# Yeicor/sdf-viewer

Measured on AMD Instinct MI355X. Metric: Mvoxels/s grid fill + Mrays/s sphere-trace @1080p, demo SDF, higher is better.
Workload: dtype f32

## Files before the change

### include/sdfgrid.h

```cpp
#ifndef SDFGRID_H
#define SDFGRID_H

#include <stddef.h>
#include <stdint.h>

#ifdef __cplusplus
extern "C" {
#endif

#define SDFV_ABI_VERSION 5

typedef enum sdfv_status {
    SDFV_OK = 0,
    SDFV_ERR_INVALID_ARGUMENT = -1,
    SDFV_ERR_UNKNOWN_SDF = -2,
    SDFV_ERR_HIP = -3,
    SDFV_ERR_NO_DEVICE = -4,
    SDFV_ERR_COMM = -5
} sdfv_status;

typedef struct sdfv_sample {
    float distance;
    float color[3];
    float metallic;
// ... 111 lines not shown
int  sdfv_camera_look_at(sdfv_camera *cam, const float eye[3], const float target[3], const float up[3],
                         float fovy_degrees, float aspect, float z_near, float z_far);


int sdfv_grid_init(const sdfv_grid *grid, float *tex0, float *tex1, void *stream);

int sdfv_grid_init_unvisited(const sdfv_grid *grid, uint32_t step, float *tex0, float *tex1, float *dist, void *stream);
int sdfv_grid_init_unvisited_ex(const sdfv_grid *grid, uint32_t step, float *tex0, float *tex1, float *dist, uint32_t flags,
                                void *stream);

int sdfv_fill_grid(const sdfv_demo_params *params, uint32_t sdf_id, const sdfv_grid *grid,
                   float *tex0, float *tex1, void *stream);

int sdfv_fill_grid_commit(const sdfv_demo_params *params, uint32_t sdf_id, const sdfv_grid *grid, float *tex0,
                          float *tex1, float *dist, void *stream);

#define SDFV_PASS_FRESH_GRID 1u
#define SDFV_PASS_SAME_LOAD  2u
#define SDFV_PASS_VIRGIN_GRID 4u
#define SDFV_PASS_VOLUME_INTERLEAVED 8u
#define SDFV_PASS_EXPECT_NOOP 16u
int sdfv_fill_grid_pass_ex(const sdfv_demo_params *params, uint32_t sdf_id, const sdfv_grid *grid, uint32_t step,
                           const float *changed_box, float *tex0, float *tex1, float *dist, uint32_t flags, void *stream);

int sdfv_pack_samples(const sdfv_grid *grid, uint64_t index_base, const uint32_t *indices, const sdfv_sample *samples, size_t n,
                      float *tex0, float *tex1, float *dist, uint32_t flags, void *stream);

size_t sdfv_emit_update_points_scratch_bytes(uint64_t n);
int sdfv_emit_update_points(const sdfv_grid *grid, uint32_t step, uint64_t cursor, uint64_t n, const float *changed_box,
                            const float *dist, uint32_t flags, float *points, uint32_t *indices, uint32_t *count, void *scratch,
// ... 284 lines not shown
```

### sdf-viewer_amd/__init__.py

```python
import ctypes as C
import os

import sys
import warnings

_hip_already_up = "torch" in sys.modules and getattr(sys.modules["torch"], "cuda", None) is not None \
    and sys.modules["torch"].cuda.is_initialized()
if "GPU_MAX_HW_QUEUES" not in os.environ:
    if _hip_already_up:
        warnings.warn("sdf-viewer_amd imported after the HIP runtime initialised: GPU_MAX_HW_QUEUES keeps its default "
                      "(4); the multi-GPU fill step may serialise its streams (DESIGN.md 6)", RuntimeWarning)
    else:
        os.environ["GPU_MAX_HW_QUEUES"] = "8"

import torch

from . import _capi
from ._capi import (Camera, DemoParams, Grid, Light, MarchAux, RenderParams, Sample, SdfvError, check, f3, lib,
                    MATERIAL_BRICK, MATERIAL_NORMAL, SDF_CUBE, SDF_DEMO, SDF_SPHERE)

AIR_DIST = lib.sdfv_air_dist()
AUX_FLOATS = C.sizeof(MarchAux) // 4


# ... 54 lines not shown
def _dev_ptr(t, what):
    if not (isinstance(t, torch.Tensor) and t.is_cuda and t.is_contiguous() and t.dtype == torch.float32):
        raise TypeError(f"{what} must be a contiguous float32 CUDA(HIP) tensor")
    return C.c_void_p(t.data_ptr())


def grid_init(grid, tex0, tex1, stream=None):
    check(lib.sdfv_grid_init(C.byref(grid), _dev_ptr(tex0, "tex0"), _dev_ptr(tex1, "tex1"), _stream_ptr(stream)))


def grid_init_unvisited(grid, step, tex0, tex1, dist=None, stream=None, flags=0):
    check(lib.sdfv_grid_init_unvisited_ex(C.byref(grid), int(step), _dev_ptr(tex0, "tex0"), _dev_ptr(tex1, "tex1"),
                                          None if dist is None else _dev_ptr(dist, "dist"), int(flags), _stream_ptr(stream)))


def fill_grid(params, grid, tex0, tex1, sdf_id=SDF_DEMO, stream=None, dist=None):
    assert tex0.numel() == slab_voxels(grid) * 4 and tex1.numel() == slab_voxels(grid) * 4
    assert dist is None or dist.numel() == slab_voxels(grid)
    check(lib.sdfv_fill_grid_commit(C.byref(params), sdf_id, C.byref(grid), _dev_ptr(tex0, "tex0"),
                                    _dev_ptr(tex1, "tex1"), None if dist is None else _dev_ptr(dist, "dist"),
                                    _stream_ptr(stream)))


def fill_grid_pass(params, grid, step, tex0, tex1, changed_box=None, sdf_id=SDF_DEMO, stream=None, dist=None, flags=0):
    box = None if changed_box is None else (C.c_float * 6)(*[float(x) for x in changed_box])
    check(lib.sdfv_fill_grid_pass_ex(C.byref(params), sdf_id, C.byref(grid), int(step), box, _dev_ptr(tex0, "tex0"),
                                     _dev_ptr(tex1, "tex1"), None if dist is None else _dev_ptr(dist, "dist"), int(flags),
                                     _stream_ptr(stream)))


def pack_samples(grid, samples, tex0, tex1, indices=None, index_base=0, dist=None, flags=0, stream=None):
    assert samples.is_cuda and samples.dtype == torch.float32 and samples.is_contiguous() and samples.shape[-1] == 7
    n = samples.numel() // 7
# ... 255 lines not shown
```

### sdf-viewer_amd/_capi.py

```python
import ctypes as C
import os

_HERE = os.path.dirname(os.path.abspath(__file__))
LIB_PATH = os.environ.get("SDFGRID_LIBRARY") or os.path.join(_HERE, "libsdfgrid.so")


class SdfvError(RuntimeError):
    def __init__(self, code, message):
        super().__init__(f"libsdfgrid error {code}: {message}")
        self.code = code


class Sample(C.Structure):
    _fields_ = [("distance", C.c_float), ("color", C.c_float * 3), ("metallic", C.c_float),
                ("roughness", C.c_float), ("occlusion", C.c_float)]


class DemoParams(C.Structure):
    _fields_ = [("cube_half_side", C.c_float), ("cube_material", C.c_uint32),
                ("sphere_radius", C.c_float), ("sphere_material", C.c_uint32),
                ("max_distance_custom_material", C.c_float), ("disable_sphere", C.c_uint32)]


class Grid(C.Structure):
# ... 75 lines not shown
    "sdfv_render_params_default": (None, [C.POINTER(RenderParams), C.POINTER(Grid)]),
    "sdfv_camera_look_at": (C.c_int, [C.POINTER(Camera), C.POINTER(C.c_float), C.POINTER(C.c_float),
                                      C.POINTER(C.c_float), C.c_float, C.c_float, C.c_float, C.c_float]),
    "sdfv_grid_init": (C.c_int, [C.POINTER(Grid), C.c_void_p, C.c_void_p, C.c_void_p]),
    "sdfv_grid_init_unvisited": (C.c_int, [C.POINTER(Grid), C.c_uint32, C.c_void_p, C.c_void_p, C.c_void_p, C.c_void_p]),
    "sdfv_grid_init_unvisited_ex": (C.c_int, [C.POINTER(Grid), C.c_uint32, C.c_void_p, C.c_void_p, C.c_void_p, C.c_uint32, C.c_void_p]),
    "sdfv_fill_grid": (C.c_int, [C.POINTER(DemoParams), C.c_uint32, C.POINTER(Grid), C.c_void_p, C.c_void_p,
                                 C.c_void_p]),
    "sdfv_pack_samples": (C.c_int, [C.POINTER(Grid), C.c_uint64, C.c_void_p, C.c_void_p, C.c_size_t, C.c_void_p, C.c_void_p,
                                    C.c_void_p, C.c_uint32, C.c_void_p]),
    "sdfv_emit_update_points_scratch_bytes": (C.c_size_t, [C.c_uint64]),
    "sdfv_emit_update_points": (C.c_int, [C.POINTER(Grid), C.c_uint32, C.c_uint64, C.c_uint64, C.POINTER(C.c_float), C.c_void_p,
                                          C.c_uint32, C.c_void_p, C.c_void_p, C.c_void_p, C.c_void_p, C.c_size_t, C.c_void_p]),
    "sdfv_fill_grid_commit": (C.c_int, [C.POINTER(DemoParams), C.c_uint32, C.POINTER(Grid), C.c_void_p, C.c_void_p,
                                        C.c_void_p, C.c_void_p]),
    "sdfv_fill_grid_pass_ex": (C.c_int, [C.POINTER(DemoParams), C.c_uint32, C.POINTER(Grid), C.c_uint32,
                                         C.POINTER(C.c_float), C.c_void_p, C.c_void_p, C.c_void_p, C.c_uint32, C.c_void_p]),
    "sdfv_sample_points": (C.c_int, [C.POINTER(DemoParams), C.c_uint32, C.c_void_p, C.c_size_t, C.c_int,
                                     C.c_void_p, C.c_void_p]),
    "sdfv_normal_points": (C.c_int, [C.POINTER(DemoParams), C.c_uint32, C.c_void_p, C.c_size_t, C.c_float,
                                     C.c_int, C.c_void_p, C.c_void_p]),
    "sdfv_commit_distance": (C.c_int, [C.POINTER(Grid), C.c_void_p, C.c_void_p, C.c_void_p]),
    "sdfv_commit_pairs": (C.c_int, [C.POINTER(Grid), C.c_void_p, C.c_void_p, C.c_void_p]),
    "sdfv_band_rows": (C.c_uint32, [C.c_uint32, C.c_uint32, C.c_uint32]),
    "sdfv_band_rows_ex": (C.c_uint32, [C.c_uint32, C.c_uint32, C.c_uint32, C.c_uint32]),
    "sdfv_march_volume_advice": (C.c_int, [C.POINTER(Grid), C.POINTER(C.c_uint32)]),
    "sdfv_commit_interleaved": (C.c_int, [C.POINTER(Grid), C.c_void_p, C.c_void_p, C.c_void_p]),
    "sdfv_fill_grid_host": (C.c_int, [C.POINTER(DemoParams), C.c_uint32, C.POINTER(Grid), C.c_void_p, C.c_void_p]),
    "sdfv_sample_points_host": (C.c_int, [C.POINTER(DemoParams), C.c_uint32, C.c_void_p, C.c_size_t, C.c_int,
                                          C.c_void_p]),
# ... 132 lines not shown
```

### sdf-viewer_amd/csrc/api_fill.hip

```cpp
#include <cstring>

#include "api_internal.h"
#include "fill_kernels.h"
#include "ingest_kernels.h"
#include "program_kernels.h"

using namespace sdfv;

namespace {

template <typename Args>
void set_grid_fill_args(Args& a, const sdfv_grid& g, float* tex0, float* tex1, float* dist = nullptr, uint32_t dist_ilv = 0) {
    a.W = g.dims[0];
    a.H = g.dims[1];
    a.z_begin = g.z_begin;
    a.slab_d = g.z_end - g.z_begin;
    sdfv::set_voxel_coords(a, g);
    a.air_dist = air_dist();
    a.tex0 = reinterpret_cast<float4*>(tex0);
    a.tex1 = reinterpret_cast<float4*>(tex1);
    a.dist = dist;
    a.dist_ilv = dist_ilv;
    a.srgb_round = g_options.ext_srgb_quant;
}
// ... 135 lines not shown
                                              grid->z_end - grid->z_begin, step, air_dist(),
                                              (flags & SDFV_PASS_VOLUME_INTERLEAVED) ? 1u : 0u, (hipStream_t)stream));
}

int sdfv_fill_grid_commit(const sdfv_demo_params* params, uint32_t sdf_id, const sdfv_grid* grid, float* tex0,
                          float* tex1, float* dist, void* stream) {
    if (int rc = check_params(params, sdf_id)) return rc;
    if (int rc = check_grid(grid)) return rc;
    if (int rc = check_textures(tex0, tex1)) return rc;
    if (int rc = check_word_aligned("dist", dist)) return rc;
    if (int rc = need_device()) return rc;
    sdfv::FillArgs a = make_fill_args(*params, sdf_id, *grid, tex0, tex1);
    a.dist = dist;
    if (int rc = check_one_launch(a)) return rc;
    SDFV_HIP_RETURN(sdfv::launch_fill_dense(a, fill_launch_config(dist != nullptr), (hipStream_t)stream));
}

int sdfv_fill_grid(const sdfv_demo_params* params, uint32_t sdf_id, const sdfv_grid* grid, float* tex0, float* tex1,
                   void* stream) {
    return sdfv_fill_grid_commit(params, sdf_id, grid, tex0, tex1, nullptr, stream);
}

int sdfv_fill_grid_pass_ex(const sdfv_demo_params* params, uint32_t sdf_id, const sdfv_grid* grid, uint32_t step,
                           const float* changed_box, float* tex0, float* tex1, float* dist, uint32_t flags, void* stream) {
    if (int rc = check_params(params, sdf_id)) return rc;
    if (int rc = check_grid(grid)) return rc;
    if (int rc = need_textures(tex0, tex1)) return rc;
    if (step == 0 || (step & (step - 1))) return set_error(SDFV_ERR_INVALID_ARGUMENT, "step %u is not a power of two", step);
    if (flags & ~(SDFV_PASS_FRESH_GRID | SDFV_PASS_SAME_LOAD | SDFV_PASS_VIRGIN_GRID | SDFV_PASS_VOLUME_INTERLEAVED | SDFV_PASS_EXPECT_NOOP))
        return set_error(SDFV_ERR_INVALID_ARGUMENT, "unknown pass flags 0x%x", flags);
// ... 119 lines not shown
```

### sdf-viewer_amd/csrc/demo_sdf_device.h

```cpp
#pragma once

#include <hip/hip_runtime.h>
#include <stdint.h>

#include "../../include/sdfgrid.h"

namespace sdfv {

__device__ __forceinline__ float fmod_pow2(float a, float m, float inv_m) {
    return a - truncf(a * inv_m) * m;
}

struct Mat {
    float r, g, b, metallic, roughness, occlusion;
};

__device__ __forceinline__ Mat brick_tex2d(float u, float v) {
    const float BRICK_WIDTH = 0.5f, BRICK_HEIGHT = 0.25f;
    const float max_cement_displacement = 0.2f / 2.0f * 0.25f;
    float row_num = v * 4.0f;
    float brick_offset = floorf(row_num) * 0.25f;
    float bx = fmod_pow2(fabsf(u + brick_offset), BRICK_WIDTH, 2.0f);
    float by = fmod_pow2(fabsf(v), BRICK_HEIGHT, 4.0f);
    bool cement = bx < max_cement_displacement || bx > BRICK_WIDTH - max_cement_displacement ||
// ... 249 lines not shown
        distance = fmaxf(d_box, -d_sph);
        float inter = fabsf(d_box) - fabsf(d_sph);
        if (fabsf(inter) <= prm.max_distance_custom_material) {
            m = PackedSet<Cfg::kRound>::kCustom;
        } else if (inter < 0.0f) {
            m = cube_packed<Cfg>(prm, px, py, pz, d_box, lut);
        } else {
            m = sphere_packed<Cfg>(prm, px, py, pz, len, d_sph, lut);
        }
    }
    t0.x = clamp01_rust(1e-1f + distance);
    t0.y = m.lr; t0.z = m.lg; t0.w = m.lb;
    t1.x = m.metallic; t1.y = m.roughness; t1.z = m.occlusion; t1.w = air_dist;
}

__device__ __forceinline__ float voxel_coord(uint32_t idx, float dim_minus_1, float bb_size, float bb_min) {
    float p = (float)idx;
    p = p / dim_minus_1;
    p = p * bb_size;
    p = p + bb_min;
    return p;
}


__device__ __forceinline__ void cube_normal(const sdfv_demo_params& prm, float px, float py, float pz,
                                            float& nx, float& ny, float& nz) {
    float side = prm.cube_half_side;
    nx = fabsf(px) > side ? signum_f32(px) : 0.0f;
    ny = fabsf(py) > side ? signum_f32(py) : 0.0f;
    nz = fabsf(pz) > side ? signum_f32(pz) : 0.0f;
// ... 45 lines not shown
```

### sdf-viewer_amd/csrc/fill_kernels.h

```cpp
#pragma once

#include <hip/hip_runtime.h>
#include <stdint.h>

#include "../../include/sdfgrid.h"

namespace sdfv {

struct FillArgs {
    sdfv_demo_params prm;
    uint32_t sdf_id;
    uint32_t W, H, D;
    uint32_t z_begin;
    uint32_t slab_d;
    float dm1[3];
    float bb_size[3];
    float bb_min[3];
    float air_dist;
    uint32_t x_chunks;
    unsigned long long w_magic;
    uint32_t z_step;
    float4* tex0;
    float4* tex1;
    float* dist;
// ... 39 lines not shown
    uint32_t no_adaptive;
    uint32_t stream_loads;
    uint64_t index_limit;
    uint32_t n_visited;
    DivU32 div_nx, div_ny, div_w;
};

struct FillLaunch {
    bool nontemporal;
    bool force_flat = false, force_rows = false;
    bool force_paired = false, force_pairrows = false;
    bool xcd_pairing = false;
};

hipError_t launch_fill_dense(const FillArgs& a, const FillLaunch& cfg, hipStream_t stream);
struct OrderedBlocks {
    uint32_t per_slice, total;
};
OrderedBlocks ordered_blocks(const FillArgs& a);
hipError_t launch_fill_dense_ordered(const FillArgs& a, uint32_t block_begin, uint32_t block_end, hipStream_t stream);
struct CopySegments {
    const float4* src[4];
    float4* dst[4];
    uint32_t n[4];
    float* r_out[4];
};
hipError_t launch_copy_segments(const CopySegments& c, hipStream_t stream);
hipError_t launch_fill_slices(const FillArgs& a, hipStream_t stream);
hipError_t launch_fill_pass(const FillArgs& a, const PassArgs& p, const FillLaunch& dense_cfg, hipStream_t stream);
hipError_t launch_commit_distance(const float* tex0, float* dist, uint64_t n_voxels, hipStream_t stream);
// ... 8 lines not shown
```

### sdf-viewer_amd/csrc/fill_kernels.hip

```cpp
#include "fill_kernels.h"

#include "kernel_common.h"

namespace sdfv {

namespace {

template <typename T>
__device__ __forceinline__ T load_scan(const T* p, uint32_t stream) {
    return stream ? load_once(p) : *p;
}

template <int TX, bool NT, typename Cfg, bool ORDERED = false>
__global__ __launch_bounds__(kBlock) void fill_dense_kernel(FillArgs a) {
    if (!ORDERED) signal_launch_started(a);
    dense_fill_rows<TX, NT, ORDERED>(a, DemoFillEval<Cfg>{a.prm, a.sdf_id});
}

template <bool NT, typename Cfg>
__global__ __launch_bounds__(kBlock) void fill_dense_pairrows_kernel(FillArgs a) {
    __shared__ float s_lut[256];
    __shared__ float2 s_yz[2];
    const uint32_t tid = threadIdx.x;
    signal_launch_started(a);
    const uint32_t pair = a.x_chunks == 1 ? blockIdx.x : blockIdx.x / a.x_chunks;
    const uint32_t chunk = blockIdx.x - pair * a.x_chunks;
    const LdsLut lut = stage_srgb_lut(s_lut);
    if (tid < 2) s_yz[tid] = stage_row_yz(a, 2 * pair + tid);
    __syncthreads();
    const uint32_t x = chunk * kBlock + tid;
    const float px = voxel_coord(x, a.dm1[0], a.bb_size[0], a.bb_min[0]);
// ... 376 lines not shown
}

template <int TX, bool NT>
hipError_t launch_dense_cfg(const FillArgs& args, hipStream_t stream) {
    constexpr int TY = kBlock / TX;
    FillArgs a = args;
    a.x_chunks = (a.W + TX - 1) / TX;
    const uint64_t n_rows = (uint64_t)a.H * a.slab_d;
    const uint64_t blocks = a.x_chunks * ((n_rows + TY - 1) / TY);
    if (blocks > 0x7fffffffull) return hipErrorInvalidValue;
    dim3 grid((uint32_t)blocks, 1, 1);
    SDFV_LAUNCH_CFG(a, (fill_dense_kernel<TX, NT, Cfg>), grid, dim3(kBlock), 0, stream, a);
    return hipGetLastError();
}

template <bool NT>
hipError_t launch_dense_pairrows(const FillArgs& args, hipStream_t stream) {
    FillArgs a = args;
    a.x_chunks = a.W / kBlock;
    const uint64_t blocks = a.x_chunks * ((uint64_t)a.H * a.slab_d / 2);
    if (blocks > 0x7fffffffull) return hipErrorInvalidValue;
    SDFV_LAUNCH_CFG(a, (fill_dense_pairrows_kernel<NT, Cfg>), dim3((uint32_t)blocks), dim3(kBlock), 0, stream, a);
    return hipGetLastError();
}

template <bool NT>
hipError_t launch_dense_ilv_paired(const FillArgs& args, hipStream_t stream) {
    FillArgs a = args;
    a.x_chunks = a.W / kBlock;
    const uint64_t units = a.x_chunks * ((uint64_t)a.H * a.slab_d / 2);
// ... 110 lines not shown
            return cfg.nontemporal ? launch_dense_ilv_paired<true>(a, stream) : launch_dense_ilv_paired<false>(a, stream);
        if (a.W % kBlock == 0 && (cfg.force_pairrows || (a.W >= 2 * kBlock && !cfg.force_rows)))
            return cfg.nontemporal ? launch_dense_pairrows<true>(a, stream) : launch_dense_pairrows<false>(a, stream);
        return a.W <= 64 ? launch_dense_tx<64>(a, cfg, stream) : launch_dense_tx<128>(a, cfg, stream);
    }
    const uint32_t chunk = a.W <= 64 ? 64 : (a.W <= 128 ? 128 : 256);
    const bool lanes_full = a.W % chunk == 0;
    const uint64_t n_vox = (uint64_t)a.W * a.H * a.slab_d;
    if (n_vox < (1ull << 32) && (cfg.force_flat || (!lanes_full && !cfg.force_rows)))
        return cfg.nontemporal ? launch_dense_flat<true>(a, stream) : launch_dense_flat<false>(a, stream);
    if (a.W <= 64) return launch_dense_tx<64>(a, cfg, stream);
    if (a.W <= 128) return launch_dense_tx<128>(a, cfg, stream);
    return launch_dense_tx<256>(a, cfg, stream);
}

static DivU32 make_div(uint32_t d) {
    DivU32 v;
    v.pow2 = d != 0 && (d & (d - 1)) == 0;
    v.shift = 0;
    while (v.pow2 && (1u << v.shift) < d) ++v.shift;
    v.magic = d > 1 ? (~0ull / d) + 1ull : 0ull;
    return v;
}

hipError_t launch_fill_pass(const FillArgs& a, const PassArgs& pass, const FillLaunch& dense_cfg, hipStream_t stream) {
    PassArgs p = pass;
    if (p.virgin) p.fresh = p.all_required = 1;
    for (int i = 0; i < 3; ++i) {
        p.approx_scale[i] = a.dm1[i] > 0.0f ? a.bb_size[i] / a.dm1[i] : 0.0f;
        p.approx_margin[i] = 64.0f * 1.1920929e-7f * (fabsf(a.bb_size[i]) + fabsf(a.bb_min[i]));
// ... 121 lines not shown
```

### sdf-viewer_amd/csrc/kernel_common.h

```cpp
#pragma once

#include <hip/hip_runtime.h>
#include <stdint.h>

#include "demo_sdf_device.h"
#include "fill_kernels.h"

namespace sdfv {

constexpr int kBlock = 256;

typedef float v4f __attribute__((ext_vector_type(4)));

namespace {
__constant__ float c_srgb_lut[256] = {
#include "srgb_lut.inc"
};
}

struct LdsLut {
    const float* p;
    __device__ __forceinline__ float operator[](uint32_t i) const { return p[i]; }
};

// ... 160 lines not shown
            store_texel<NT>(a.tex1 + o, v1);
            if (a.dist && !ilv) a.dist[o] = v0.x;
        }
    }
    if (ilv) {
        __shared__ float s_d[kBlock];
        s_d[tid] = v0.x;
        __syncthreads();
        if ((ty & 1u) == 0 && in_range)
            reinterpret_cast<float2*>(a.dist)[(uint64_t)(row >> 1) * a.W + x] = make_float2(s_d[tid], s_d[tid + TX]);
    }
    if constexpr (ORDERED)
        if (ob.boundary) store_staged(a, ob, o, v0, v1);
}

template <typename Cfg>
struct DemoFillEval {
    const sdfv_demo_params& prm;
    uint32_t sdf_id;
    __device__ __forceinline__ void operator()(float px, float py, float pz, const LdsLut& lut, float air_dist, float4& t0,
                                               float4& t1) const {
        fill_voxel<Cfg>(prm, sdf_id, px, py, pz, lut, air_dist, t0, t1);
    }
};

inline uint32_t blocks_for(size_t n) { return (uint32_t)((n + kBlock - 1) / kBlock); }

template <typename Staged, typename Scalar>
hipError_t launch_staged_then_tail(size_t n, bool aligned, Staged&& staged, Scalar&& scalar) {
    if (n == 0) return hipSuccess;
    const size_t whole = aligned ? n / kBlock : 0;
    const size_t done = whole * kBlock;
    const size_t tail_blocks = (n - done + kBlock - 1) / kBlock;
    if (whole > 0x7fffffffull || tail_blocks > 0x7fffffffull) return hipErrorInvalidValue;
    if (whole > 0) staged((uint32_t)whole);
    if (done < n) scalar((uint32_t)tail_blocks, done);
    return hipGetLastError();
// ... 4 lines not shown
```

### sdf-viewer_amd/host/host_capi.cpp

```cpp
#include <hip/hip_runtime_api.h>

#include <chrono>
#include <cstring>
#include <memory>
#include <string>
#include <vector>

#include <sstream>

#include "loading_manager.hpp"
#include "mesh.hpp"
#include "program_sdf.hpp"
#include "provider_sdf.hpp"
#include "sdf_demo.hpp"
#include "scene.hpp"
#include "sdf_viewer.hpp"

using namespace sdfviewer;

#pragma GCC visibility push(default)
extern "C" {

void* sdfvh_lm_new(size_t lx, size_t ly, size_t lz, size_t passes) { return new LoadingManager({lx, ly, lz}, passes); }
void sdfvh_lm_free(void* m) { delete static_cast<LoadingManager*>(m); }
// ... 176 lines not shown
    if (rc != 0) return rc;
    if (hipStreamSynchronize((hipStream_t)V(v).stream) != hipSuccess) return -1;
    return hipMemcpy(rgba_host, out.get(), out.bytes(), hipMemcpyDeviceToHost) == hipSuccess ? 0 : -1;
}

int sdfvh_viewer_render_device(void* v, uint32_t width, uint32_t height, const float eye[3], float* rgba_device) {
    Camera cam;
    if (eye) cam.position = Vec3{eye[0], eye[1], eye[2]};
    cam.set_viewport(width, height);
    return V(v).material.render(cam, rgba_device, nullptr, V(v).stream);
}
int sdfvh_viewer_pairs_valid(void* v) {
    if (V(v).material.dist && V(v).material.dist_interleaved) return V(v).material.lod_dist_between_samples == 1.0f ? 2 : 0;
    return V(v).material.pairs && V(v).material.pairs_valid ? (V(v).material.pairs_interleaved ? 2 : 1) : 0;
}
int sdfvh_viewer_sync(void* v) { return hipStreamSynchronize((hipStream_t)V(v).stream) == hipSuccess ? 0 : -1; }

struct SceneHandle {
    long long now_ms = 0;
    std::unique_ptr<SDFViewerAppScene> scene;
};
void* sdfvh_scene_new(void* sdf) {
    auto* h = new SceneHandle();
    auto clock = [h] { return std::chrono::steady_clock::time_point(std::chrono::milliseconds(h->now_ms)); };
    h->scene.reset(new SDFViewerAppScene(*static_cast<std::shared_ptr<SDFSurface>*>(sdf), clock));
    if (!h->scene->sdf_viewer) {
        delete h;
        return nullptr;
    }
    return h;
// ... 91 lines not shown
```

### sdf-viewer_amd/host/sdf_viewer.cpp

```cpp
#include "sdf_viewer.hpp"

#include <hip/hip_runtime_api.h>

#include <cmath>
#include <cstdio>
#include <cstring>

namespace sdfviewer {

DeviceBuffer::DeviceBuffer(size_t bytes) : bytes_(bytes) {
    if (bytes && hipMalloc(&ptr_, bytes) != hipSuccess) {
        (void)hipGetLastError();
        ptr_ = nullptr;
    }
}
DeviceBuffer::~DeviceBuffer() {
    if (owned_ && ptr_) (void)hipFree(ptr_);
}
DeviceBuffer& DeviceBuffer::operator=(DeviceBuffer&& o) noexcept {
    if (this != &o) {
        if (owned_ && ptr_) (void)hipFree(ptr_);
        ptr_ = o.ptr_;
        bytes_ = o.bytes_;
        owned_ = o.owned_;
// ... 98 lines not shown
    std::unique_ptr<SDFViewer> v(new SDFViewer(voxels, bb, loading_passes));
    if (!v->material.tex0->ok() || !v->material.tex1->ok()) return nullptr;
    v->material.undefined_rows = true;
    v->material.defined_step = 0;
    v->material.dist = std::make_shared<DeviceBuffer>(v->material.tex0->bytes() / 4);
    v->dist_synced_ = v->material.dist->ok();
    if (!v->dist_synced_) v->material.dist.reset();
    if (v->dist_synced_ && layout == VolumeLayout::Auto) {
        const sdfv_grid g = v->grid();
        uint32_t kind = SDFV_MARCH_VOLUME_NONE;
        if (sdfv_march_volume_advice(&g, &kind) == 0 && kind == SDFV_MARCH_VOLUME_INTERLEAVED) v->material.dist_interleaved = true;
    } else if (v->dist_synced_ && layout == VolumeLayout::Interleaved) {
        if (voxels[1] & 1) return nullptr;
        v->material.dist_interleaved = true;
    }
    return v;
}

sdfv_grid SDFViewer::grid() const {
    sdfv_grid g;
    for (int i = 0; i < 3; ++i) g.dims[i] = material.tex_size[i];
    g.bb_min[0] = bounding_box[0].x; g.bb_min[1] = bounding_box[0].y; g.bb_min[2] = bounding_box[0].z;
    g.bb_max[0] = bounding_box[1].x; g.bb_max[1] = bounding_box[1].y; g.bb_max[2] = bounding_box[1].z;
    g.z_begin = 0;
    g.z_end = g.dims[2];
    return g;
}

size_t SDFViewer::update(SDFSurface& sdf, std::chrono::nanoseconds max_delta_time) {
    error_.clear();
    visited_before_throw_ = 0;
    bool just_changed_box = false;
    if (const auto dev_now = sdf.device_sdf()) {
        if (!load_sdf_ || memcmp(&*load_sdf_, &*dev_now, sizeof(*dev_now)) != 0) {
            if (!fresh_) same_load_ = false;
            load_sdf_ = *dev_now;
        }
    }
    if (auto new_box = sdf.changed()) {
        same_load_ = false;
        changed_box = changed_box ? merge_bounding_boxes(*changed_box, *new_box) : *new_box;
// ... 25 lines not shown
            const float dm1 = (float)g.dims[i] - 1.0f, size = g.bb_max[i] - g.bb_min[i];
            float first = 0.0f / dm1;
            first = first * size;
            first = first + g.bb_min[i];
            float last = ((float)g.dims[i] - 1.0f) / dm1;
            last = last * size;
            last = last + g.bb_min[i];
            if (!(first >= lo[i] && first <= hi[i] && last >= lo[i] && last <= hi[i])) return false;
        }
        return true;
    };
    const bool all_passes_fit = loading_mgr.total_iterations() == 0 && loading_mgr.step_size() != 0 &&
                                max_delta_time >= std::chrono::milliseconds(1);
    if (all_passes_fit && ((fresh_ && !changed_box) || box_covers_grid())) {
        float* dist_out = dist_synced_ ? material.dist->f32() : nullptr;
        int rc;
        if (dist_out && material.dist_interleaved) {
            float box[6];
            const float* box_ptr = nullptr;
            uint32_t flags = SDFV_PASS_VOLUME_INTERLEAVED;
            if (changed_box) {
                box[0] = (*changed_box)[0].x; box[1] = (*changed_box)[0].y; box[2] = (*changed_box)[0].z;
                box[3] = (*changed_box)[1].x; box[4] = (*changed_box)[1].y; box[5] = (*changed_box)[1].z;
                box_ptr = box;
                if (material.materialize(stream) != 0) {
                    error_ = sdfv_last_error();
                    return 0;
                }
            } else {
                flags |= (material.undefined_rows ? SDFV_PASS_VIRGIN_GRID : SDFV_PASS_FRESH_GRID) | SDFV_PASS_SAME_LOAD;
            }
            rc = sdfv_fill_grid_pass_ex(&dev->params, dev->sdf_id, &g, 1u, box_ptr, tex0_device(), tex1_device(), dist_out, flags, stream);
        } else {
            rc = sdfv_fill_grid_commit(&dev->params, dev->sdf_id, &g, tex0_device(), tex1_device(), dist_out, stream);
        }
        if (rc != 0) {
            error_ = sdfv_last_error();
            return 0;
        }
        fresh_ = false;
        material.undefined_rows = false;
        material.pairs_valid = false;
        while (loading_mgr.step_size() != 0) loading_mgr.finish_pass();
        loaded_once_ = true;
        publish_lod();
        return loading_mgr.total_iterations() - start_iter;
    }
    bool first = true;
    while (first || std::chrono::steady_clock::now() - start_time < max_delta_time) {
        first = false;
        const size_t step = loading_mgr.step_size();
        if (step == 0) break;
        float box[6];
        const float* box_ptr = nullptr;
        if (changed_box) {
            box[0] = (*changed_box)[0].x; box[1] = (*changed_box)[0].y; box[2] = (*changed_box)[0].z;
            box[3] = (*changed_box)[1].x; box[4] = (*changed_box)[1].y; box[5] = (*changed_box)[1].z;
            box_ptr = box;
        }
        uint32_t flags = 0;
        if (same_load_ && !changed_box)
            flags = material.undefined_rows ? (SDFV_PASS_VIRGIN_GRID | SDFV_PASS_SAME_LOAD)
                                            : ((fresh_ ? SDFV_PASS_FRESH_GRID : 0u) | SDFV_PASS_SAME_LOAD);
        else if (material.materialize(stream) != 0) {
            error_ = sdfv_last_error();
            break;
        }
        if (dist_synced_ && material.dist_interleaved) flags |= SDFV_PASS_VOLUME_INTERLEAVED;
        if (loaded_once_ && !changed_box && flags == (flags & SDFV_PASS_VOLUME_INTERLEAVED)) flags |= SDFV_PASS_EXPECT_NOOP;
        if (sdfv_fill_grid_pass_ex(&dev->params, dev->sdf_id, &g, (uint32_t)step, box_ptr, tex0_device(), tex1_device(),
                                   dist_synced_ ? material.dist->f32() : nullptr, flags, stream) != 0) {
            error_ = sdfv_last_error();
            break;
        }
        fresh_ = false;
        if (material.undefined_rows) {
            material.defined_step = (uint32_t)step;
            if (step == 1) material.undefined_rows = false;
        }
        material.pairs_valid = false;
        loading_mgr.finish_pass();
        if (loading_mgr.step_size() == 0) loaded_once_ = true;
        publish_lod();
    }
    return loading_mgr.total_iterations() - start_iter;
}

void SDFViewer::publish_lod() {
    material.lod_dist_between_samples = std::pow(2.0f, (float)(uint8_t)loading_mgr.passes_left());
}

void SDFViewer::commit() {
    publish_lod();
    if (dist_synced_ && material.dist_interleaved) return;
    if (dist_synced_ && loading_mgr.step_size() == 0 && !material.pairs_valid) {
        const sdfv_grid g = grid();
        if (!material.pairs && !material.no_march_volume) {
            uint32_t kind = SDFV_MARCH_VOLUME_PAIRS;
            (void)sdfv_march_volume_advice(&g, &kind);
            material.pairs_interleaved = kind == SDFV_MARCH_VOLUME_INTERLEAVED;
            material.no_march_volume = kind == SDFV_MARCH_VOLUME_NONE;
            if (!material.no_march_volume)
                material.pairs = std::make_shared<DeviceBuffer>(material.dist->bytes() * (material.pairs_interleaved ? 1 : 2));
        }
        if (!material.pairs) return;
        const int rc = !material.pairs->ok() ? -1
                       : material.pairs_interleaved ? sdfv_commit_interleaved(&g, material.dist->f32(), material.pairs->f32(), stream)
                                                    : sdfv_commit_pairs(&g, material.dist->f32(), material.pairs->f32(), stream);
        if (rc == 0)
            material.pairs_valid = true;
// ... 17 lines not shown
```

### sdf-viewer_amd/host/sdf_viewer.hpp

```cpp
#pragma once

#include <chrono>
#include <memory>
#include <optional>

#include "loading_manager.hpp"
#include "sdf_surface.hpp"

namespace sdfviewer {

struct Camera {
    Vec3 position{2.5f, 3.0f, 5.0f};
    Vec3 target{0.0f, 0.0f, 0.0f};
    Vec3 up{0.0f, 1.0f, 0.0f};
    float fovy_degrees = 45.0f;
    float z_near = 0.1f, z_far = 1000.0f;
    uint32_t viewport_width = 0, viewport_height = 0;
    static Camera new_perspective(uint32_t width, uint32_t height, Vec3 position, Vec3 target, Vec3 up,
                                  float fovy_degrees, float z_near, float z_far);
    void set_viewport(uint32_t width, uint32_t height) {
        viewport_width = width;
        viewport_height = height;
    }
    sdfv_camera to_device() const;
// ... 15 lines not shown
    bool ok() const { return ptr_ != nullptr || bytes_ == 0; }

   private:
    void* ptr_ = nullptr;
    size_t bytes_ = 0;
    bool owned_ = true;
};

struct SDFViewerMaterial {
    std::shared_ptr<DeviceBuffer> tex0;
    std::shared_ptr<DeviceBuffer> tex1;
    std::shared_ptr<DeviceBuffer> dist;
    bool dist_interleaved = false;
    std::shared_ptr<DeviceBuffer> pairs;
    bool pairs_valid = false;
    bool no_march_volume = false;
    bool pairs_interleaved = false;
    mutable bool undefined_rows = false;
    mutable uint32_t defined_step = 0;
    int materialize(void* stream) const;
    std::array<uint32_t, 3> tex_size{0, 0, 0};
    BoundingBox voxels_bounds;
    float lod_dist_between_samples = 1.0f;
    float color[4] = {1.0f, 1.0f, 1.0f, 1.0f};
    float gamma = 0.0f;

    sdfv_render_params uniforms() const;
    int render(const Camera& camera, float* rgba_device, sdfv_march_aux* aux_device, void* stream) const;
};

// ... 19 lines not shown
    float* tex0_device() const { return material.tex0->f32(); }
    float* tex1_device() const { return material.tex1->f32(); }
    int download(float* tex0_host, float* tex1_host) const;
    const char* last_error() const { return error_.c_str(); }
    size_t visited_before_throw() const { return visited_before_throw_; }

    SDFViewerMaterial material;
    LoadingManager loading_mgr;
    BoundingBox bounding_box;
    std::optional<BoundingBox> changed_box;
    bool changed_box_while_loading = false;
    void* stream = nullptr;

   private:
    SDFViewer(std::array<size_t, 3> voxels, const BoundingBox& bb, size_t passes);
    size_t update_host(SDFSurface& sdf, std::chrono::nanoseconds max_delta_time);
    size_t update_device(SDFSurface& sdf, std::chrono::nanoseconds max_delta_time);
    struct DeviceRuns;
    struct DeviceRunsDeleter {
        void operator()(DeviceRuns* p) const;
    };
    struct Ingest;
    struct IngestDeleter {
        void operator()(Ingest* p) const;
    };
    std::unique_ptr<Ingest, IngestDeleter> ingest_;
    bool host_mirror_valid_ = false;
    std::string error_;
    bool fresh_ = true;
    bool loaded_once_ = false;
// ... 10 lines not shown
```

### sdf-viewer_amd/host/sdf_viewer_device.cpp

```cpp
#include <hip/hip_runtime_api.h>

#include <algorithm>
#include <exception>

#include "sdf_viewer.hpp"

namespace sdfviewer {

namespace {
constexpr size_t kFirstRun = 4096;
constexpr size_t kDefaultCapacity = 1u << 23;
constexpr size_t kCostSamples = 4096;
}

struct SDFViewer::DeviceRuns {
    DeviceBuffer points, indices, samples, count, scratch;
    uint32_t* h_count = nullptr;
    size_t capacity = 0;
    const SDFSurface* cost_sdf = nullptr;
    double sample_cost = 0.0;
    ~DeviceRuns() {
        if (h_count) (void)hipHostFree(h_count);
    }
    bool reserve(size_t n) {
// ... 37 lines not shown
    host_mirror_valid_ = false;
    if (material.materialize(stream) != 0) {
        error_ = sdfv_last_error();
        return 0;
    }
    if (!device_runs_) device_runs_.reset(new DeviceRuns());
    DeviceRuns& dr = *device_runs_;
    if (!dr.reserve(ingest_capacity ? ingest_capacity : std::min(n_voxels, kDefaultCapacity))) {
        error_ = "cannot allocate the device-sampled load's buffers";
        return 0;
    }
    same_load_ = false;
    load_sdf_.reset();
    fresh_ = false;
    material.pairs_valid = false;

    const uint32_t flags = material.dist_interleaved ? SDFV_PASS_VOLUME_INTERLEAVED : 0u;
    float* dist = material.dist->f32();
    float box[6];
    const float* box_ptr = nullptr;
    if (changed_box) {
        box[0] = (*changed_box)[0].x; box[1] = (*changed_box)[0].y; box[2] = (*changed_box)[0].z;
        box[3] = (*changed_box)[1].x; box[4] = (*changed_box)[1].y; box[5] = (*changed_box)[1].z;
        box_ptr = box;
    }
    if (dr.cost_sdf != &sdf) {
        dr.cost_sdf = &sdf;
        dr.sample_cost = 0.0;
    }
    auto fail_run = [&](const char* what) {
// ... 68 lines not shown
```

### sdf-viewer_amd/host/sdf_viewer_ingest.cpp

```cpp
#include <hip/hip_runtime_api.h>

#include <algorithm>
#include <cstring>
#include <exception>
#include <thread>
#include <vector>

#include "sdf_viewer.hpp"
#include "worker_pool.hpp"

namespace sdfviewer {

namespace {

inline float clamp01_rust(float v) { return v < 0.0f ? 0.0f : (v > 1.0f ? 1.0f : v); }

constexpr size_t kGather = 2048;

}

struct SDFViewer::Ingest {
    struct Buffer {
        sdfv_sample* samples = nullptr;
        uint32_t* indices = nullptr;
// ... 115 lines not shown
    for (int a = 0; a < 3; ++a) {
        in.coords[a].resize(g.dims[a]);
        const float dm1 = (float)g.dims[a] - 1.0f, size = bbmax[a] - bbmin[a];
        for (uint32_t i = 0; i < g.dims[a]; ++i) {
            float p = (float)i;
            p = p / dm1;
            p = p * size;
            p = p + bbmin[a];
            in.coords[a][i] = p;
        }
    }
    same_load_ = false;
    load_sdf_.reset();
    fresh_ = false;
    material.pairs_valid = false;

    const uint32_t pack_flags = (dist_synced_ && material.dist_interleaved) ? SDFV_PASS_VOLUME_INTERLEAVED : 0u;
    float* dist_dev = dist_synced_ ? material.dist->f32() : nullptr;
    const bool has_box = changed_box.has_value();
    const BoundingBox box = has_box ? *changed_box : BoundingBox{};
    if (has_box) in.journal.resize(in.capacity);
    if (in.cost_sdf != &sdf) {
        in.cost_sdf = &sdf;
        in.record_cost = 0.0;
    }
    const auto deadline = max_delta_time < std::chrono::hours(24 * 365) ? start_time + max_delta_time
                                                                        : std::chrono::steady_clock::time_point::max();

    struct Run {
        Ingest::Buffer* b = nullptr;
// ... 175 lines not shown
```

Before: 204,100.

## Fuse march pair-volume construction into the dense grid fill kernel

Adds a dense fill kernel that writes the (distance, upper-neighbour distance) pair volume alongside the textures and distance volume. Neighbours come from shared memory within the block, and the row past the block edge is recomputed with a distance-only SDF evaluation. The host now allocates the pair buffer ahead of time and marks it written, so the separate commit-pairs pass after loading is skipped. This saves a full read of the distance volume and a separate launch, but the fused kernel uses more shared memory, adds a barrier and does extra SDF evaluations for one row per block.

```diff
diff --git a/include/sdfgrid.h b/include/sdfgrid.h
--- a/include/sdfgrid.h
+++ b/include/sdfgrid.h
@@ -149,6 +149,8 @@
 
 int sdfv_fill_grid_commit(const sdfv_demo_params *params, uint32_t sdf_id, const sdfv_grid *grid, float *tex0,
                           float *tex1, float *dist, void *stream);
+int sdfv_fill_grid_commit_pairs(const sdfv_demo_params *params, uint32_t sdf_id, const sdfv_grid *grid, float *tex0,
+                                float *tex1, float *dist, float *pairs, void *stream);
 
 #define SDFV_PASS_FRESH_GRID 1u
 #define SDFV_PASS_SAME_LOAD  2u
diff --git a/sdf-viewer_amd/__init__.py b/sdf-viewer_amd/__init__.py
--- a/sdf-viewer_amd/__init__.py
+++ b/sdf-viewer_amd/__init__.py
@@ -92,9 +92,15 @@
                                           None if dist is None else _dev_ptr(dist, "dist"), int(flags), _stream_ptr(stream)))
 
 
-def fill_grid(params, grid, tex0, tex1, sdf_id=SDF_DEMO, stream=None, dist=None):
+def fill_grid(params, grid, tex0, tex1, sdf_id=SDF_DEMO, stream=None, dist=None, pairs=None):
     assert tex0.numel() == slab_voxels(grid) * 4 and tex1.numel() == slab_voxels(grid) * 4
     assert dist is None or dist.numel() == slab_voxels(grid)
+    if pairs is not None:
+        assert pairs.numel() == slab_voxels(grid) * 2
+        check(lib.sdfv_fill_grid_commit_pairs(C.byref(params), sdf_id, C.byref(grid), _dev_ptr(tex0, "tex0"), _dev_ptr(tex1, "tex1"),
+                                              None if dist is None else _dev_ptr(dist, "dist"), _dev_ptr(pairs, "pairs"),
+                                              _stream_ptr(stream)))
+        return
     check(lib.sdfv_fill_grid_commit(C.byref(params), sdf_id, C.byref(grid), _dev_ptr(tex0, "tex0"),
                                     _dev_ptr(tex1, "tex1"), None if dist is None else _dev_ptr(dist, "dist"),
                                     _stream_ptr(stream)))
diff --git a/sdf-viewer_amd/_capi.py b/sdf-viewer_amd/_capi.py
--- a/sdf-viewer_amd/_capi.py
+++ b/sdf-viewer_amd/_capi.py
@@ -113,6 +113,8 @@
                                           C.c_uint32, C.c_void_p, C.c_void_p, C.c_void_p, C.c_void_p, C.c_size_t, C.c_void_p]),
     "sdfv_fill_grid_commit": (C.c_int, [C.POINTER(DemoParams), C.c_uint32, C.POINTER(Grid), C.c_void_p, C.c_void_p,
                                         C.c_void_p, C.c_void_p]),
+    "sdfv_fill_grid_commit_pairs": (C.c_int, [C.POINTER(DemoParams), C.c_uint32, C.POINTER(Grid), C.c_void_p, C.c_void_p,
+                                              C.c_void_p, C.c_void_p, C.c_void_p]),
     "sdfv_fill_grid_pass_ex": (C.c_int, [C.POINTER(DemoParams), C.c_uint32, C.POINTER(Grid), C.c_uint32,
                                          C.POINTER(C.c_float), C.c_void_p, C.c_void_p, C.c_void_p, C.c_uint32, C.c_void_p]),
     "sdfv_sample_points": (C.c_int, [C.POINTER(DemoParams), C.c_uint32, C.c_void_p, C.c_size_t, C.c_int,
diff --git a/sdf-viewer_amd/csrc/api_fill.hip b/sdf-viewer_amd/csrc/api_fill.hip
--- a/sdf-viewer_amd/csrc/api_fill.hip
+++ b/sdf-viewer_amd/csrc/api_fill.hip
@@ -173,6 +173,22 @@
     a.dist = dist;
     if (int rc = check_one_launch(a)) return rc;
     SDFV_HIP_RETURN(sdfv::launch_fill_dense(a, fill_launch_config(dist != nullptr), (hipStream_t)stream));
+}
+
+int sdfv_fill_grid_commit_pairs(const sdfv_demo_params* params, uint32_t sdf_id, const sdfv_grid* grid, float* tex0,
+                                float* tex1, float* dist, float* pairs, void* stream) {
+    if (!pairs) return sdfv_fill_grid_commit(params, sdf_id, grid, tex0, tex1, dist, stream);
+    if (int rc = check_params(params, sdf_id)) return rc;
+    if (int rc = check_grid(grid)) return rc;
+    if (int rc = check_textures(tex0, tex1)) return rc;
+    if (!dist) return set_error(SDFV_ERR_INVALID_ARGUMENT, "the pair volume is written next to the distance volume: dist is NULL");
+    if (int rc = check_word_aligned("dist", dist)) return rc;
+    if ((uintptr_t)pairs & 7) return set_error(SDFV_ERR_INVALID_ARGUMENT, "pairs must be 8-byte aligned");
+    if (int rc = need_device()) return rc;
+    sdfv::FillArgs a = make_fill_args(*params, sdf_id, *grid, tex0, tex1);
+    a.dist = dist;
+    if (int rc = check_one_launch(a)) return rc;
+    SDFV_HIP_RETURN(sdfv::launch_fill_dense_pairs(a, pairs, fill_launch_config(true), (hipStream_t)stream));
 }
 
 int sdfv_fill_grid(const sdfv_demo_params* params, uint32_t sdf_id, const sdfv_grid* grid, float* tex0, float* tex1,
diff --git a/sdf-viewer_amd/csrc/demo_sdf_device.h b/sdf-viewer_amd/csrc/demo_sdf_device.h
--- a/sdf-viewer_amd/csrc/demo_sdf_device.h
+++ b/sdf-viewer_amd/csrc/demo_sdf_device.h
@@ -287,6 +287,22 @@
     t1.x = m.metallic; t1.y = m.roughness; t1.z = m.occlusion; t1.w = air_dist;
 }
 
+template <typename Cfg>
+__device__ __forceinline__ float fill_distance(const sdfv_demo_params& prm, uint32_t sdf_id_rt, float px, float py, float pz) {
+    const uint32_t sdf_id = Cfg::sdf_id(sdf_id_rt);
+    float distance;
+    if (sdf_id == SDFV_SDF_CUBE || (sdf_id == SDFV_SDF_DEMO && Cfg::disable_sphere(prm))) {
+        distance = cube_distance(prm, px, py, pz);
+    } else if (sdf_id == SDFV_SDF_SPHERE) {
+        distance = vec_length(px, py, pz) - prm.sphere_radius;
+    } else {
+        const float d_box = cube_distance(prm, px, py, pz);
+        const float d_sph = vec_length(px, py, pz) - prm.sphere_radius;
+        distance = fmaxf(d_box, -d_sph);
+    }
+    return clamp01_rust(1e-1f + distance);
+}
+
 __device__ __forceinline__ float voxel_coord(uint32_t idx, float dim_minus_1, float bb_size, float bb_min) {
     float p = (float)idx;
     p = p / dim_minus_1;
diff --git a/sdf-viewer_amd/csrc/fill_kernels.h b/sdf-viewer_amd/csrc/fill_kernels.h
--- a/sdf-viewer_amd/csrc/fill_kernels.h
+++ b/sdf-viewer_amd/csrc/fill_kernels.h
@@ -77,6 +77,7 @@
 };
 
 hipError_t launch_fill_dense(const FillArgs& a, const FillLaunch& cfg, hipStream_t stream);
+hipError_t launch_fill_dense_pairs(const FillArgs& a, float* pairs, const FillLaunch& cfg, hipStream_t stream);
 struct OrderedBlocks {
     uint32_t per_slice, total;
 };
diff --git a/sdf-viewer_amd/csrc/fill_kernels.hip b/sdf-viewer_amd/csrc/fill_kernels.hip
--- a/sdf-viewer_amd/csrc/fill_kernels.hip
+++ b/sdf-viewer_amd/csrc/fill_kernels.hip
@@ -15,6 +15,12 @@
 __global__ __launch_bounds__(kBlock) void fill_dense_kernel(FillArgs a) {
     if (!ORDERED) signal_launch_started(a);
     dense_fill_rows<TX, NT, ORDERED>(a, DemoFillEval<Cfg>{a.prm, a.sdf_id});
+}
+
+template <int TX, bool NT, typename Cfg>
+__global__ __launch_bounds__(kBlock) void fill_dense_pairs_kernel(FillArgs a, float2* pairs) {
+    signal_launch_started(a);
+    dense_fill_rows_pairs<TX, NT>(a, pairs, DemoFillEval<Cfg>{a.prm, a.sdf_id});
 }
 
 template <bool NT, typename Cfg>
@@ -421,6 +427,23 @@
     return hipGetLastError();
 }
 
+template <int TX>
+hipError_t launch_dense_pairs_tx(const FillArgs& args, float* pairs, bool nt, hipStream_t stream) {
+    constexpr int ROWS = kBlock / TX;
+    FillArgs a = args;
+    a.x_chunks = a.W / TX;
+    const uint64_t n_rows = (uint64_t)a.H * a.slab_d;
+    const uint64_t blocks = a.x_chunks * ((n_rows + ROWS - 1) / ROWS);
+    if (blocks > 0x7fffffffull) return hipErrorInvalidValue;
+    float2* p2 = reinterpret_cast<float2*>(pairs);
+    if (nt) {
+        SDFV_LAUNCH_CFG(a, (fill_dense_pairs_kernel<TX, true, Cfg>), dim3((uint32_t)blocks), dim3(kBlock), 0, stream, a, p2);
+    } else {
+        SDFV_LAUNCH_CFG(a, (fill_dense_pairs_kernel<TX, false, Cfg>), dim3((uint32_t)blocks), dim3(kBlock), 0, stream, a, p2);
+    }
+    return hipGetLastError();
+}
+
 template <bool NT>
 hipError_t launch_dense_pairrows(const FillArgs& args, hipStream_t stream) {
     FillArgs a = args;
@@ -561,6 +584,20 @@
     return launch_dense_tx<256>(a, cfg, stream);
 }
 
+hipError_t launch_fill_dense_pairs(const FillArgs& a, float* pairs, const FillLaunch& cfg, hipStream_t stream) {
+    if (a.W == 0 || a.H == 0 || a.slab_d == 0) return hipSuccess;
+    if (!a.dist || a.dist_ilv || !pairs || ((uintptr_t)pairs & 7)) return hipErrorInvalidValue;
+    const uint32_t chunk = a.W <= 64 ? 64 : (a.W <= 128 ? 128 : 256);
+    const uint64_t n_rows = (uint64_t)a.H * a.slab_d, n_vox = n_rows * a.W;
+    if (a.W % chunk != 0 || cfg.force_flat || cfg.force_rows || n_rows >= (1ull << 32)) {
+        if (hipError_t e = launch_fill_dense(a, cfg, stream)) return e;
+        return launch_commit_pairs(a.dist, pairs, a.W, a.H, n_vox, stream);
+    }
+    if (chunk == 64) return launch_dense_pairs_tx<64>(a, pairs, cfg.nontemporal, stream);
+    if (chunk == 128) return launch_dense_pairs_tx<128>(a, pairs, cfg.nontemporal, stream);
+    return launch_dense_pairs_tx<256>(a, pairs, cfg.nontemporal, stream);
+}
+
 static DivU32 make_div(uint32_t d) {
     DivU32 v;
     v.pow2 = d != 0 && (d & (d - 1)) == 0;
diff --git a/sdf-viewer_amd/csrc/kernel_common.h b/sdf-viewer_amd/csrc/kernel_common.h
--- a/sdf-viewer_amd/csrc/kernel_common.h
+++ b/sdf-viewer_amd/csrc/kernel_common.h
@@ -198,6 +198,59 @@
         if (ob.boundary) store_staged(a, ob, o, v0, v1);
 }
 
+template <int TX, bool NT, typename Args, typename Eval>
+__device__ __forceinline__ void dense_fill_rows_pairs(const Args& a, float2* __restrict__ pairs, const Eval& eval) {
+    constexpr int TY = kBlock / TX;
+    __shared__ float s_lut[256];
+    __shared__ float2 s_yz[TY + 1];
+    __shared__ uint32_t s_top[TY];
+    __shared__ float s_d[TY > 1 ? kBlock : 1];
+
+    const uint32_t tid = threadIdx.x;
+    const uint32_t n_rows = a.H * a.slab_d;
+    const uint32_t row_group = a.x_chunks == 1 ? blockIdx.x : blockIdx.x / a.x_chunks;
+    const uint32_t chunk = blockIdx.x - row_group * a.x_chunks;
+    const uint32_t row0 = row_group * TY;
+    const LdsLut lut = stage_srgb_lut(s_lut);
+    if (tid <= TY && row0 + tid < n_rows) {
+        s_yz[tid] = stage_row_yz(a, row0 + tid);
+        if (tid < TY) s_top[tid] = (row0 + tid + 1) % a.H == 0 ? 1u : 0u;
+    }
+    __syncthreads();
+
+    const uint32_t tx = tid % TX, ty = tid / TX;
+    const uint32_t x = chunk * TX + tx;
+    const uint32_t row = row0 + ty;
+    const bool in_range = x < a.W && row < n_rows;
+    const uint64_t o = (uint64_t)row * a.W + x;
+    const float px = voxel_coord(x, a.dm1[0], a.bb_size[0], a.bb_min[0]);
+    float d = 0.0f;
+    if (in_range) {
+        const float2 yz = s_yz[ty];
+        float4 v0, v1;
+        eval(px, yz.x, yz.y, lut, a.air_dist, v0, v1);
+        store_texel<NT>(a.tex0 + o, v0);
+        store_texel<NT>(a.tex1 + o, v1);
+        a.dist[o] = v0.x;
+        d = v0.x;
+    }
+    if constexpr (TY > 1) {
+        s_d[tid] = d;
+        __syncthreads();
+    }
+    if (!in_range) return;
+    float up = d;
+    if (!s_top[ty]) {
+        if (TY > 1 && ty + 1 < TY) {
+            up = s_d[tid + TX];
+        } else {
+            const float2 yz = s_yz[TY];
+            up = eval.distance(px, yz.x, yz.y);
+        }
+    }
+    pairs[o] = make_float2(d, up);
+}
+
 template <typename Cfg>
 struct DemoFillEval {
     const sdfv_demo_params& prm;
@@ -205,6 +258,9 @@
     __device__ __forceinline__ void operator()(float px, float py, float pz, const LdsLut& lut, float air_dist, float4& t0,
                                                float4& t1) const {
         fill_voxel<Cfg>(prm, sdf_id, px, py, pz, lut, air_dist, t0, t1);
+    }
+    __device__ __forceinline__ float distance(float px, float py, float pz) const {
+        return fill_distance<Cfg>(prm, sdf_id, px, py, pz);
     }
 };
 
diff --git a/sdf-viewer_amd/host/host_capi.cpp b/sdf-viewer_amd/host/host_capi.cpp
--- a/sdf-viewer_amd/host/host_capi.cpp
+++ b/sdf-viewer_amd/host/host_capi.cpp
@@ -214,6 +214,19 @@
     if (V(v).material.dist && V(v).material.dist_interleaved) return V(v).material.lod_dist_between_samples == 1.0f ? 2 : 0;
     return V(v).material.pairs && V(v).material.pairs_valid ? (V(v).material.pairs_interleaved ? 2 : 1) : 0;
 }
+int sdfvh_viewer_download_volumes(void* v, float* dist_host, float* pairs_host) {
+    const SDFViewerMaterial& m = V(v).material;
+    if (hipStreamSynchronize((hipStream_t)V(v).stream) != hipSuccess) return -1;
+    if (dist_host && (!m.dist || hipMemcpy(dist_host, m.dist->get(), m.dist->bytes(), hipMemcpyDeviceToHost) != hipSuccess)) return -1;
+    if (pairs_host && (!m.pairs || hipMemcpy(pairs_host, m.pairs->get(), m.pairs->bytes(), hipMemcpyDeviceToHost) != hipSuccess)) return -1;
+    return m.pairs && m.pairs_written ? 1 : 0;
+}
+int sdfvh_viewer_poke_pairs(void* v, size_t index, float value) {
+    const SDFViewerMaterial& m = V(v).material;
+    if (!m.pairs || (index + 1) * sizeof(float) > m.pairs->bytes()) return -1;
+    if (hipStreamSynchronize((hipStream_t)V(v).stream) != hipSuccess) return -1;
+    return hipMemcpy(m.pairs->f32() + index, &value, sizeof(float), hipMemcpyHostToDevice) == hipSuccess ? 0 : -1;
+}
 int sdfvh_viewer_sync(void* v) { return hipStreamSynchronize((hipStream_t)V(v).stream) == hipSuccess ? 0 : -1; }
 
 struct SceneHandle {
diff --git a/sdf-viewer_amd/host/sdf_viewer.cpp b/sdf-viewer_amd/host/sdf_viewer.cpp
--- a/sdf-viewer_amd/host/sdf_viewer.cpp
+++ b/sdf-viewer_amd/host/sdf_viewer.cpp
@@ -136,6 +136,7 @@
         if (voxels[1] & 1) return nullptr;
         v->material.dist_interleaved = true;
     }
+    (void)v->pairs_for_fill();
     return v;
 }
 
@@ -147,6 +148,23 @@
     g.z_begin = 0;
     g.z_end = g.dims[2];
     return g;
+}
+
+float* SDFViewer::pairs_for_fill() {
+    if (!dist_synced_ || material.dist_interleaved || material.no_march_volume) return nullptr;
+    if (!material.pairs) {
+        const sdfv_grid g = grid();
+        uint32_t kind = SDFV_MARCH_VOLUME_NONE;
+        if (sdfv_march_volume_advice(&g, &kind) != 0 || kind != SDFV_MARCH_VOLUME_PAIRS) return nullptr;
+        material.pairs = std::make_shared<DeviceBuffer>(material.dist->bytes() * 2);
+        material.pairs_interleaved = false;
+        if (!material.pairs->ok()) {
+            material.pairs.reset();
+            material.no_march_volume = true;
+            return nullptr;
+        }
+    }
+    return material.pairs_interleaved ? nullptr : material.pairs->f32();
 }
 
 size_t SDFViewer::update(SDFSurface& sdf, std::chrono::nanoseconds max_delta_time) {
@@ -202,6 +220,7 @@
                                 max_delta_time >= std::chrono::milliseconds(1);
     if (all_passes_fit && ((fresh_ && !changed_box) || box_covers_grid())) {
         float* dist_out = dist_synced_ ? material.dist->f32() : nullptr;
+        float* pairs_out = nullptr;
         int rc;
         if (dist_out && material.dist_interleaved) {
             float box[6];
@@ -220,7 +239,8 @@
             }
             rc = sdfv_fill_grid_pass_ex(&dev->params, dev->sdf_id, &g, 1u, box_ptr, tex0_device(), tex1_device(), dist_out, flags, stream);
         } else {
-            rc = sdfv_fill_grid_commit(&dev->params, dev->sdf_id, &g, tex0_device(), tex1_device(), dist_out, stream);
+            pairs_out = pairs_for_fill();
+            rc = sdfv_fill_grid_commit_pairs(&dev->params, dev->sdf_id, &g, tex0_device(), tex1_device(), dist_out, pairs_out, stream);
         }
         if (rc != 0) {
             error_ = sdfv_last_error();
@@ -229,6 +249,7 @@
         fresh_ = false;
         material.undefined_rows = false;
         material.pairs_valid = false;
+        material.pairs_written = pairs_out != nullptr;
         while (loading_mgr.step_size() != 0) loading_mgr.finish_pass();
         loaded_once_ = true;
         publish_lod();
@@ -256,8 +277,12 @@
         }
         if (dist_synced_ && material.dist_interleaved) flags |= SDFV_PASS_VOLUME_INTERLEAVED;
         if (loaded_once_ && !changed_box && flags == (flags & SDFV_PASS_VOLUME_INTERLEAVED)) flags |= SDFV_PASS_EXPECT_NOOP;
-        if (sdfv_fill_grid_pass_ex(&dev->params, dev->sdf_id, &g, (uint32_t)step, box_ptr, tex0_device(), tex1_device(),
-                                   dist_synced_ ? material.dist->f32() : nullptr, flags, stream) != 0) {
+        float* pairs_out = step == 1 && (flags & SDFV_PASS_SAME_LOAD) ? pairs_for_fill() : nullptr;
+        const int rc = pairs_out ? sdfv_fill_grid_commit_pairs(&dev->params, dev->sdf_id, &g, tex0_device(), tex1_device(),
+                                                               material.dist->f32(), pairs_out, stream)
+                                 : sdfv_fill_grid_pass_ex(&dev->params, dev->sdf_id, &g, (uint32_t)step, box_ptr, tex0_device(),
+                                                          tex1_device(), dist_synced_ ? material.dist->f32() : nullptr, flags, stream);
+        if (rc != 0) {
             error_ = sdfv_last_error();
             break;
         }
@@ -267,6 +292,7 @@
             if (step == 1) material.undefined_rows = false;
         }
         material.pairs_valid = false;
+        material.pairs_written = pairs_out != nullptr;
         loading_mgr.finish_pass();
         if (loading_mgr.step_size() == 0) loaded_once_ = true;
         publish_lod();
@@ -282,6 +308,10 @@
     publish_lod();
     if (dist_synced_ && material.dist_interleaved) return;
     if (dist_synced_ && loading_mgr.step_size() == 0 && !material.pairs_valid) {
+        if (material.pairs && material.pairs_written) {
+            material.pairs_valid = true;
+            return;
+        }
         const sdfv_grid g = grid();
         if (!material.pairs && !material.no_march_volume) {
             uint32_t kind = SDFV_MARCH_VOLUME_PAIRS;
diff --git a/sdf-viewer_amd/host/sdf_viewer.hpp b/sdf-viewer_amd/host/sdf_viewer.hpp
--- a/sdf-viewer_amd/host/sdf_viewer.hpp
+++ b/sdf-viewer_amd/host/sdf_viewer.hpp
@@ -53,6 +53,7 @@
     bool dist_interleaved = false;
     std::shared_ptr<DeviceBuffer> pairs;
     bool pairs_valid = false;
+    bool pairs_written = false;
     bool no_march_volume = false;
     bool pairs_interleaved = false;
     mutable bool undefined_rows = false;
@@ -102,6 +103,7 @@
 
    private:
     SDFViewer(std::array<size_t, 3> voxels, const BoundingBox& bb, size_t passes);
+    float* pairs_for_fill();
     size_t update_host(SDFSurface& sdf, std::chrono::nanoseconds max_delta_time);
     size_t update_device(SDFSurface& sdf, std::chrono::nanoseconds max_delta_time);
     struct DeviceRuns;
diff --git a/sdf-viewer_amd/host/sdf_viewer_device.cpp b/sdf-viewer_amd/host/sdf_viewer_device.cpp
--- a/sdf-viewer_amd/host/sdf_viewer_device.cpp
+++ b/sdf-viewer_amd/host/sdf_viewer_device.cpp
@@ -75,6 +75,7 @@
     load_sdf_.reset();
     fresh_ = false;
     material.pairs_valid = false;
+    material.pairs_written = false;
 
     const uint32_t flags = material.dist_interleaved ? SDFV_PASS_VOLUME_INTERLEAVED : 0u;
     float* dist = material.dist->f32();
diff --git a/sdf-viewer_amd/host/sdf_viewer_ingest.cpp b/sdf-viewer_amd/host/sdf_viewer_ingest.cpp
--- a/sdf-viewer_amd/host/sdf_viewer_ingest.cpp
+++ b/sdf-viewer_amd/host/sdf_viewer_ingest.cpp
@@ -153,6 +153,7 @@
     load_sdf_.reset();
     fresh_ = false;
     material.pairs_valid = false;
+    material.pairs_written = false;
 
     const uint32_t pack_flags = (dist_synced_ && material.dist_interleaved) ? SDFV_PASS_VOLUME_INTERLEAVED : 0u;
     float* dist_dev = dist_synced_ ? material.dist->f32() : nullptr;
```

Measured after the change: 204,100. No clear change (-0.0%).
